# MAGIC-SCAN/adipose_tissue-unet

Measured on AMD Instinct MI355X. Metric: 1024^2 tiles/sec (train), higher is better.
Workload: dtype bf16; 1 GPU; unet_bn L5 base64 1024x1024x3 bf16 B=4/GPU (BASELINE configs[2]); preset=unet_bn, levels=5, tile=1024, batch_per_gpu=4, global_batch=4, parallelism=dp1

## Files before the change

adipose_tissue-unet_amd/csrc/conv_common.h:

```cpp
#pragma once
#include "workspace.h"

struct FwdArgs {
  const void* srcA; const void* srcB;
  const float* scA; const float* shA;
  const float* scB; const float* shB;
  int CAs, CBs;
  int Nimg, Hs, Ws;
  int up;
  int Ho, Wo, stride;
  int kh, kw, dil, pad;
  const void* W; int Kpad; int K;
  const float* bias;
  int Nout;
  int relu;
  uint32_t drop_seed; float drop_rate;
  void* out; int out_stride; int out_mode; int Cps;
  void* out2; int out2_stride; int split_c;
  const void* addend; int addend_stride;
  const void* mask; int mask_stride; float mask_scale;
  const void* mask2; int mask2_stride; float mask2_scale;
  float* accum; int accum_stride;
  float* bn_sum; float* bn_sq;
  const void* bnr_z; int bnr_zs;
// ... 197 lines not shown
    }
    Grp<TO> gr;
    if (a.out_mode == 1) {
      int sub = n / a.Cps, c = n - sub * a.Cps;
      int nimg = m / HWo, rem = m - nimg * HWo, yo = rem / a.Wo, xo = rem - yo * a.Wo;
      size_t pix = ((size_t)nimg * (2 * a.Ho) + 2 * yo + (sub >> 1)) * (2 * a.Wo) + 2 * xo + (sub & 1);
      if constexpr (F8) {
        if (a.out_f8) {
          *reinterpret_cast<uint2*>(reinterpret_cast<unsigned char*>(a.out) + pix * a.out_stride + c) = f8x8_from_f(v);
          continue;
        }
      }
      grp_from_f(gr, v);
      grp_store(gr, reinterpret_cast<TO*>(a.out) + pix * a.out_stride + c);
    } else if (a.out_mode == 2 && n >= a.split_c) {
      const int c = n - a.split_c;
      if (a.mask2) {
        float mk[8];
        grp_load(gr, reinterpret_cast<const TO*>(a.mask2) + (size_t)m * a.mask2_stride + c);
        grp_to_f(gr, mk);
#pragma unroll
        for (int j = 0; j < 8; ++j) v[j] = mk[j] > 0.f ? v[j] * a.mask2_scale : 0.f;
      }
      grp_from_f(gr, v);
      grp_store(gr, reinterpret_cast<TO*>(a.out2) + (size_t)m * a.out2_stride + c);
      if (a.bn_sum) {
#pragma unroll
        for (int j = 0; j < 8; ++j) { bs[j] += v[j]; bq[j] += v[j] * v[j]; }
      }
      continue;
    } else {
      if (!a.out) continue;
      if constexpr (F8) {
        if (a.out_f8) {
          *reinterpret_cast<uint2*>(reinterpret_cast<unsigned char*>(a.out) + (size_t)m * a.out_stride + n) =
              f8x8_from_f(v);
          continue;
        }
      }
      float f[8];
      if (a.addend) {
        grp_load(gr, reinterpret_cast<const TO*>(a.addend) + (size_t)m * a.addend_stride + n);
        grp_to_f(gr, f);
#pragma unroll
        for (int j = 0; j < 8; ++j) v[j] += f[j];
      }
      if (a.mask) {
        grp_load(gr, reinterpret_cast<const TO*>(a.mask) + (size_t)m * a.mask_stride + n);
        grp_to_f(gr, f);
#pragma unroll
        for (int j = 0; j < 8; ++j) v[j] = f[j] > 0.f ? v[j] * a.mask_scale : 0.f;
      }
      grp_from_f(gr, v);
      grp_store(gr, reinterpret_cast<TO*>(a.out) + (size_t)m * a.out_stride + n);
      if (a.accum) {
        float* ap = a.accum + (size_t)m * a.accum_stride + n;
        float r[8];
        grp_to_f(gr, r);
#pragma unroll
        for (int j = 0; j < 8; ++j) ap[j] += r[j];
      }
    }
    if (a.bn_sum) {
#pragma unroll
      for (int j = 0; j < 8; ++j) { bs[j] += v[j]; bq[j] += v[j] * v[j]; }
    }
  }
}

template <int NTH, int BN, typename TO = bf16>
ADP_DEV void epi_rows_bnr(const FwdArgs& a, const float* tile, int rows, int m0, int n0, int tid,
                          float (&bs)[8], float (&bq)[8]) {
  constexpr int LT = BN + 4;
  constexpr int GPR = BN / 8;
  constexpr int RSTEP = NTH / GPR;
  const int cg = tid % GPR;
  const int n = n0 + cg * 8;
  if (n >= a.Nout) return;
  for (int row = tid / GPR; row < rows; row += RSTEP) {
    const int m = m0 + row;
    if (m >= a.M) break;
    float v[8], f[8];
    const float4* tp = reinterpret_cast<const float4*>(tile + row * LT + cg * 8);
    float4 t0 = tp[0], t1 = tp[1];
    v[0] = t0.x; v[1] = t0.y; v[2] = t0.z; v[3] = t0.w; v[4] = t1.x; v[5] = t1.y; v[6] = t1.z; v[7] = t1.w;
    Grp<TO> gr;
    if (a.addend) {
      grp_load(gr, reinterpret_cast<const TO*>(a.addend) + (size_t)m * a.addend_stride + n);
      grp_to_f(gr, f);
#pragma unroll
      for (int j = 0; j < 8; ++j) v[j] += f[j];
    }
    if (a.mask) {
      grp_load(gr, reinterpret_cast<const TO*>(a.mask) + (size_t)m * a.mask_stride + n);
      grp_to_f(gr, f);
#pragma unroll
      for (int j = 0; j < 8; ++j) v[j] = f[j] > 0.f ? v[j] * a.mask_scale : 0.f;
    }
    grp_from_f(gr, v);
    grp_store(gr, reinterpret_cast<TO*>(a.out) + (size_t)m * a.out_stride + n);
    grp_to_f(gr, v);
    if (ADP_DBG(a) & 8192) grp_zero(gr);
    else grp_load(gr, reinterpret_cast<const TO*>(a.bnr_z) + (size_t)m * a.bnr_zs + n);
    grp_to_f(gr, f);
    if (ADP_DBG(a) & 16384) continue;
#pragma unroll
    for (int h = 0; h < 2; ++h) {
      const float4 sc = *reinterpret_cast<const float4*>(a.bnr_sc + n + 4 * h);
      const float4 sh = *reinterpret_cast<const float4*>(a.bnr_sh + n + 4 * h);
      const float4 mu = *reinterpret_cast<const float4*>(a.bnr_mean + n + 4 * h);
      const float4 is = *reinterpret_cast<const float4*>(a.bnr_invstd + n + 4 * h);
      const float scv[4] = {sc.x, sc.y, sc.z, sc.w}, shv[4] = {sh.x, sh.y, sh.z, sh.w};
      const float muv[4] = {mu.x, mu.y, mu.z, mu.w}, isv[4] = {is.x, is.y, is.z, is.w};
#pragma unroll
      for (int j = 0; j < 4; ++j) {
        const int jj = 4 * h + j;
        const float db = fmaf(f[jj], scv[j], shv[j]) > 0.f ? v[jj] : 0.f;
        bs[jj] += db;
        bq[jj] += db * (f[jj] - muv[j]) * isv[j];
      }
    }
  }
}

template <int NTH, int BN>
ADP_DEV void epi_bn_flush(const FwdArgs& a, float* red, int n0, int tid, const float (&bs)[8],
                          const float (&bq)[8]) {
  constexpr int GPR = BN / 8;
  if (ADP_DBG(a) & 2) return;
  ADP_LDS_BARRIER();
#pragma unroll
  for (int j = 0; j < 8; ++j) { red[tid * 16 + j] = bs[j]; red[tid * 16 + 8 + j] = bq[j]; }
  ADP_LDS_BARRIER();
  if (tid < BN) {
    const int gg = tid >> 3, j = tid & 7;
    float s = 0.f, q = 0.f;
    for (int t = gg; t < NTH; t += GPR) { s += red[t * 16 + j]; q += red[t * 16 + 8 + j]; }
    const int nn = n0 + tid;
    if (nn < a.Nout) {
      const int c = a.out_mode == 1 ? nn % a.Cps : nn;
      const unsigned blk = blockIdx.x + blockIdx.y * gridDim.x;
      double* rep = a.stat + (size_t)(blk & (adp::STAT_REPL - 1)) * 2 * adp::STAT_CMAX;
      atomicAdd(rep + c, (double)s);
      atomicAdd(rep + adp::STAT_CMAX + c, (double)q);
    }
  }
}

}

namespace adp {
int launch_fwd_tap64(FwdArgs& a, hipStream_t s);
int launch_fwd_tap64p(FwdArgs& a, hipStream_t s, int tile);
int launch_fwd_halo(FwdArgs& a, hipStream_t s);
int launch_fwd_w4(FwdArgs& a, hipStream_t s);
int launch_fwd_cin8(FwdArgs& a, hipStream_t s);
int launch_fwd_cin8_f32(FwdArgs& a, hipStream_t s);
int launch_fwd_halop_f8(FwdArgs& a, hipStream_t s);
int launch_wgrad_tap64(WgradArgs& a, hipStream_t s);
int launch_wgrad_f32(WgradArgs& a, hipStream_t s);
bool wgrad_bna_fusable(const WgradArgs& a);
}
```

adipose_tissue-unet_amd/csrc/conv_igemm.hip:

```cpp
#include "conv_common.h"
#include <type_traits>

namespace {

constexpr int BM = 128, BN = 64, BK = 32, NT = 256;

template <typename T> struct LdsTr;
template <> struct LdsTr<bf16> { static constexpr int LDK = BK + 8; };
template <> struct LdsTr<float> { static constexpr int LDK = BK + 4; };


template <typename T>
ADP_DEV void load_a_group(const FwdArgs& a, Grp<T>& g, bool rowvalid, int n, int ybase, int xbase,
                          int tap, int ci, int k) {
  grp_zero(g);
  if (!rowvalid || k >= a.K) return;
  int ty = tap / a.kw, tx = tap - ty * a.kw;
  int yi = ybase + ty * a.dil - a.pad;
  int xi = xbase + tx * a.dil - a.pad;
  int Hv = a.Hs * a.up, Wv = a.Ws * a.up;
  if (yi < 0 || xi < 0 || yi >= Hv || xi >= Wv) return;
  if (a.up == 2) { yi >>= 1; xi >>= 1; }
  size_t pix = ((size_t)n * a.Hs + yi) * a.Ws + xi;
  const float* sc; const float* sh;
// ... 898 lines not shown
      Grp<T> gr;
      float f[8];
      grp_load(gr, x + m * stride + g * 8);
      grp_to_f(gr, f);
#pragma unroll
      for (int j = 0; j < 8; ++j) s[j] += f[j];
    }
  }
  __shared__ float red[NT * 8];
#pragma unroll
  for (int j = 0; j < 8; ++j) red[threadIdx.x * 8 + j] = s[j];
  __syncthreads();
  for (int c = threadIdx.x; c < C; c += NT) {
    float t = 0.f;
    for (int l = 0; l < lanes; ++l) t += red[(l * G + (c >> 3)) * 8 + (c & 7)];
    if (part) out[(size_t)blockIdx.x * C + c] = t;
    else atomicAdd(out + (fold ? c % fold : c), t);
  }
}

template <typename T>
void launch_bias_grad(const WgradArgs& a, hipStream_t s) {
  const size_t Mp = a.dy_mode == 0 ? (size_t)a.M : (size_t)a.M * 4;
  const int C = a.dy_mode == 0 ? a.Nout : a.Cps;
  const int G = C / 8, lanes = NT / G;
  const int blocks = (int)std::min<size_t>((Mp + lanes - 1) / lanes, 1024);
  const adp::Slabs part = adp::option("wgrad_det", 1) && C % 4 == 0
                              ? adp::reduce_part(adp::Slot::BiasRows, (size_t)blocks * C * sizeof(float), s)
                              : adp::Slabs{};
  hipLaunchKernelGGL(channel_sum_kernel<T>, dim3(blocks), dim3(NT), 0, s, Mp, C, a.dy_stride,
                     reinterpret_cast<const T*>(a.dY), part.p ? part.p : a.dB, 0, part.p ? 1 : 0);
  if (part.p) adp::slab_reduce(blocks, (size_t)C / 4, part, a.dB, s);
}

}

#include "../../include/adipose_hip.h"

namespace {
template <typename T>
int launch_fwd_plain(FwdArgs& a, hipStream_t s, int fast);

void fill_fwd_args(const adp_conv_desc* d, const adp_conv_io* io, FwdArgs& a) {
  a = FwdArgs{};
  a.srcA = io->srcA; a.srcB = io->srcB;
  a.scA = io->bn_scaleA; a.shA = io->bn_shiftA; a.scB = io->bn_scaleB; a.shB = io->bn_shiftB;
  a.CAs = d->CA_stride; a.CBs = d->CB_stride;
  a.Nimg = d->N; a.Hs = d->Hs; a.Ws = d->Ws; a.up = d->upsample ? 2 : 1;
  a.Ho = d->Ho; a.Wo = d->Wo; a.stride = d->stride;
  a.kh = d->kh; a.kw = d->kw; a.dil = d->dil; a.pad = d->pad;
  a.W = io->W; a.K = d->kh * d->kw * (d->CA_stride + d->CB_stride); a.Kpad = (a.K + 31) / 32 * 32;
  a.bias = io->bias; a.Nout = d->Nout; a.relu = d->relu;
  a.drop_seed = d->dropout_seed; a.drop_rate = d->dropout_rate;
  a.out = io->out; a.out_stride = d->out_stride; a.out_mode = d->out_mode; a.Cps = d->shuffle_c;
  a.out2 = io->out2; a.out2_stride = d->out2_stride; a.split_c = d->split_c;
  a.addend = io->addend; a.addend_stride = d->out_stride;
  a.mask = io->mask; a.mask_stride = d->mask_stride; a.mask_scale = d->mask_scale;
  a.mask2 = io->mask2; a.mask2_stride = d->mask2_stride; a.mask2_scale = d->mask2_scale;
  a.accum = io->accum; a.accum_stride = d->accum_stride;
  a.bn_sum = io->bn_sum; a.bn_sq = io->bn_sqsum;
  a.defer_fold = d->bn_defer_fold && io->bn_sum && !io->bnr_z;
  a.bnr_z = io->bnr_z; a.bnr_zs = d->bnr_stride;
  a.bnr_sc = io->bnr_scale; a.bnr_sh = io->bnr_shift; a.bnr_mean = io->bnr_mean; a.bnr_invstd = io->bnr_invstd;
  a.bnr_dgamma = io->bnr_dgamma; a.bnr_dbeta = io->bnr_dbeta;
  a.M = d->N * d->Ho * d->Wo;
  a.debug_flags = adp::option("fwd_debug", 0);
  a.f32 = 0;
  a.stat = (a.bn_sum || a.bnr_z) ? adp::stat_scratch() : nullptr;
  a.act_out = io->act_outA;
  a.ca_real = d->CA_real;
  auto tail48 = [](int stride, int real) { return stride == 64 && real > 0 && real <= 48; };
  a.ztail = (tail48(d->CA_stride, d->CA_real) && (d->CB_stride == 0 || tail48(d->CB_stride, d->CB_real)) ? 1 : 0) |
            (tail48(d->Nout, d->Nout_real) && d->out_mode == 0 ? 2 : 0);
}

int fold_stats(const FwdArgs& a, hipStream_t s) {
  if (!a.stat) return 0;
  if (a.defer_fold)
    return adp::defer_fold_begin(a.out_mode == 1 ? a.Cps : a.Nout, a.bn_sum, s);
  const int C = a.out_mode == 1 ? a.Cps : a.Nout;
  if (a.bnr_z) return adp::stat_fold(C, a.bnr_dbeta, a.bnr_dgamma, s);
  return adp::stat_fold(C, a.bn_sum, a.bn_sq, s);
}

int launch_fwd_f8(const adp_conv_desc* d, const adp_conv_io* io, hipStream_t s) {
  FwdArgs a;
  fill_fwd_args(d, io, a);
  a.f8 = 1;
  a.wscale = io->w_scale;
  a.out_f8 = d->out_fp8;
  ADP_REQUIRE(a.wscale && a.M > 0 && a.Nout > 0 && a.Nout % 8 == 0, "adp_conv_fwd(fp8): needs w_scale and Nout % 8 == 0");
  ADP_REQUIRE(!a.scA && !a.scB && !a.addend && !a.mask && !a.accum && !a.bn_sum && !a.bnr_z && a.drop_rate == 0.f &&
                  (d->out_mode == 0 || d->out_mode == 1) && a.out,
              "adp_conv_fwd(fp8): plain or pixel-shuffle store only (no BN / addend / mask / accum / dropout)");
  ADP_REQUIRE(d->out_mode != 1 || (d->shuffle_c > 0 && d->Nout % d->shuffle_c == 0), "adp_conv_fwd: bad shuffle_c");
  if (a.CAs == 64 && a.CBs % 64 == 0 && adp::launch_fwd_halop_f8(a, s)) {
    adp::kernel_end();
    return adp::check_launch("adp_conv_fwd");
  }
  ADP_REQUIRE(a.CAs % 128 == 0 && a.CBs % 128 == 0,
              "adp_conv_fwd(fp8): source channel strides must be multiples of 128 (one 128-channel K step per tap)");
  if (!adp::launch_fwd_tap64(a, s)) {
    adp::set_error("adp_conv_fwd(fp8): no fp8 kernel for this geometry (needs K == taps * Cin_s, K % 128 == 0)");
    return -1;
  }
  adp::kernel_end();
  return adp::check_launch("adp_conv_fwd");
}

template <typename T>
int launch_fwd(const adp_conv_desc* d, const adp_conv_io* io, hipStream_t s) {
  FwdArgs a;
  fill_fwd_args(d, io, a);
  ADP_REQUIRE(a.CAs % 8 == 0 && a.CBs % 8 == 0, "adp_conv_fwd: channel strides must be multiples of 8");
  if (d->out_fp8) {
    ADP_REQUIRE((std::is_same<T, bf16>::value), "adp_conv_fwd: out_fp8 needs a bf16 or fp8 launch");
    a.out_f8 = 1;
    if (!adp::launch_fwd_cin8(a, s)) {
      adp::set_error("adp_conv_fwd: out_fp8 on a bf16 launch: input layers only (one 8-channel source, Nout == 64, "
                     "no statistics)");
      return -1;
    }
    adp::kernel_end();
    return adp::check_launch("adp_conv_fwd");
  }
  ADP_REQUIRE(a.M > 0 && a.Nout > 0, "adp_conv_fwd: empty problem");
  ADP_REQUIRE(d->out_mode != 1 || (d->shuffle_c > 0 && d->Nout % d->shuffle_c == 0), "adp_conv_fwd: bad shuffle_c");
  ADP_REQUIRE(d->out_mode != 2 || (io->out2 && d->split_c > 0), "adp_conv_fwd: split store needs out2/split_c");
  ADP_REQUIRE(!a.bnr_z || (d->out_mode == 0 && !a.bn_sum && a.bnr_sc && a.bnr_sh && a.bnr_mean && a.bnr_invstd &&
                           a.bnr_dgamma && a.bnr_dbeta && a.bnr_zs == a.out_stride && a.bnr_zs % 8 == 0 &&
                           a.Nout % 8 == 0),
              "adp_conv_fwd: fused BN-backward reduction needs out_mode 0, all bnr_* pointers, z stride == out stride");
  ADP_REQUIRE(!(a.bn_sum || a.bnr_z) || a.stat,
              std::string("adp_conv_fwd: BatchNorm accumulator replicas unavailable: ") + adp_last_error());
  ADP_REQUIRE(!a.stat || (d->out_mode == 1 ? d->shuffle_c : d->Nout) <= adp::STAT_CMAX,
              "adp_conv_fwd: BatchNorm sums need <= 2048 channels");
  const int fast = adp::option("conv_fast", 2);
  if (a.act_out) {
    ADP_REQUIRE(a.scA && a.shA && !a.scB && a.CBs == 0 && io->srcA != io->act_outA,
                "adp_conv_fwd: act_outA needs bn_scaleA / bn_shiftA, one source and its own buffer");
    if (std::is_same<T, bf16>::value && fast == 2 && adp::launch_fwd_halo(a, s)) {
      adp::kernel_end();
      if (adp::check_launch("adp_conv_fwd")) return -2;
      return fold_stats(a, s);
    }
    const int rc = adp_bn_apply(std::is_same<T, bf16>::value ? ADP_BF16 : ADP_F32, (size_t)a.Nimg * a.Hs * a.Ws, a.CAs,
                                a.srcA, a.scA, a.shA, a.act_out, (adp_stream_t)s);
    if (rc) return rc;
    a.srcA = a.act_out;
    a.scA = a.shA = nullptr;
    a.act_out = nullptr;
  }
  if (std::is_same<T, bf16>::value && fast == 2 && !a.scA && !a.scB &&
      (adp::launch_fwd_cin8(a, s) || adp::launch_fwd_halo(a, s) || adp::launch_fwd_tap64(a, s))) {
    adp::kernel_end();
    if (adp::check_launch("adp_conv_fwd")) return -2;
    return fold_stats(a, s);
  }
  if (std::is_same<T, float>::value && fast == 2 && !a.scA && !a.scB) {
    a.f32 = 1;
    if (adp::launch_fwd_cin8_f32(a, s) || adp::launch_fwd_tap64(a, s)) {
      adp::kernel_end();
      if (adp::check_launch("adp_conv_fwd")) return -2;
      return fold_stats(a, s);
    }
    a.f32 = 0;
  }
  const FwdArgs bnr = a;
  a.bnr_z = nullptr;
  if (!a.bn_sum) a.stat = nullptr;
  const int rc = launch_fwd_plain<T>(a, s, fast);
  if (rc != 0) return rc;
  if (a.stat && fold_stats(a, s) != 0) return -2;
  if (!bnr.bnr_z) return 0;
  return adp_bn_bwd_reduce(std::is_same<T, bf16>::value ? ADP_BF16 : ADP_F32, (size_t)bnr.M, bnr.out_stride, bnr.out,
                           bnr.bnr_z, bnr.bnr_sc, bnr.bnr_sh, bnr.bnr_mean, bnr.bnr_invstd, bnr.bnr_dgamma,
                           bnr.bnr_dbeta, (adp_stream_t)s);
}

template <typename T>
int launch_fwd_plain(FwdArgs& a, hipStream_t s, int fast) {
  if (std::is_same<T, bf16>::value && fast == 2 && !a.scA && !a.scB) {
    const int w64 = (a.Nout + 63) / 64 * 64 - a.Nout, w128 = (a.Nout + 127) / 128 * 128 - a.Nout;
    if (a.Nout > 64 && w128 <= w64) {
      a.ntile_n = (a.Nout + 127) / 128;
      a.nblocks = ((a.M + 127) / 128) * a.ntile_n;
      adp::set_kernel("igemm_fwd_glds_kernel<128, 128>");
      hipLaunchKernelGGL((igemm_fwd_glds_kernel<128, 128>), dim3(a.nblocks), dim3(NT), 0, s, a);
    } else {
      a.ntile_n = (a.Nout + 63) / 64;
      a.nblocks = ((a.M + 255) / 256) * a.ntile_n;
      adp::set_kernel("igemm_fwd_glds_kernel<256, 64>");
      hipLaunchKernelGGL((igemm_fwd_glds_kernel<256, 64>), dim3(a.nblocks), dim3(NT), 0, s, a);
    }
    adp::kernel_end();
    return adp::check_launch("adp_conv_fwd");
  }
  if (std::is_same<T, bf16>::value && fast >= 1) {
    const int w64 = (a.Nout + 63) / 64 * 64 - a.Nout, w128 = (a.Nout + 127) / 128 * 128 - a.Nout;
    if (a.Nout > 64 && w128 <= w64) {
      a.ntile_n = (a.Nout + 127) / 128;
      a.nblocks = ((a.M + 127) / 128) * a.ntile_n;
      adp::set_kernel("igemm_fwd_bf16_kernel<128, 128>");
      hipLaunchKernelGGL((igemm_fwd_bf16_kernel<128, 128>), dim3(a.nblocks), dim3(NT), 0, s, a);
    } else {
      a.ntile_n = (a.Nout + 63) / 64;
      a.nblocks = ((a.M + 255) / 256) * a.ntile_n;
      adp::set_kernel("igemm_fwd_bf16_kernel<256, 64>");
      hipLaunchKernelGGL((igemm_fwd_bf16_kernel<256, 64>), dim3(a.nblocks), dim3(NT), 0, s, a);
    }
    adp::kernel_end();
    return adp::check_launch("adp_conv_fwd");
  }
  a.ntile_n = (a.Nout + BN - 1) / BN;
  const int ntm = (a.M + BM - 1) / BM;
  a.nblocks = ntm * a.ntile_n;
  adp::set_kernel(std::is_same<T, bf16>::value ? "igemm_fwd_kernel<bf16>" : "igemm_fwd_kernel<float>");
  hipLaunchKernelGGL(igemm_fwd_kernel<T>, dim3(a.nblocks), dim3(NT), 0, s, a);
  adp::kernel_end();
  return adp::check_launch("adp_conv_fwd");
}

template <typename T>
int launch_wgrad(const adp_conv_desc* d, const adp_conv_io* io, const void* dY, int dy_stride,
                 float* dW, float* dB, hipStream_t s, const adp_bn_bwd_args* bn = nullptr) {
  WgradArgs a{};
  a.srcA = io->srcA; a.srcB = io->srcB;
  a.scA = io->bn_scaleA; a.shA = io->bn_shiftA; a.scB = io->bn_scaleB; a.shB = io->bn_shiftB;
  a.CAs = d->CA_stride; a.CBs = d->CB_stride; a.Nimg = d->N; a.Hs = d->Hs; a.Ws = d->Ws;
  a.up = d->upsample ? 2 : 1; a.Ho = d->Ho; a.Wo = d->Wo; a.stride = d->stride;
  a.kh = d->kh; a.kw = d->kw; a.dil = d->dil; a.pad = d->pad;
  a.K = d->kh * d->kw * (d->CA_stride + d->CB_stride); a.Kpad = (a.K + 31) / 32 * 32;
  a.dY = dY; a.dy_stride = dy_stride; a.dy_mode = d->out_mode == 1 ? 1 : 0; a.Cps = d->shuffle_c;
  a.Nout = d->Nout; a.dW = dW; a.dB = dB;
  a.M = d->N * d->Ho * d->Wo;
  a.ca_real = d->CA_real; a.cb_real = d->CB_real; a.nout_real = d->Nout_real;
  ADP_REQUIRE(a.CAs % 8 == 0 && a.CBs % 8 == 0 && a.Nout % 8 == 0,
              "adp_conv_wgrad: channel strides and Nout must be multiples of 8");
  ADP_REQUIRE(d->out_mode != 2, "adp_conv_wgrad: split-store descriptors are dgrad-only");
  if (bn) {
    a.bna_dA = bn->dA; a.bna_z = bn->z;
    a.bna_sc = bn->scale; a.bna_sh = bn->shift; a.bna_mean = bn->mean; a.bna_invstd = bn->invstd;
    a.bna_gamma = bn->gamma; a.bna_dgamma = bn->dgamma; a.bna_dbeta = bn->dbeta;
    a.bna_inv_count = 1.f / bn->count;
    if (!(std::is_same<T, bf16>::value && adp::option("conv_fast", 2) == 2 && adp::wgrad_bna_fusable(a))) {
      a.bna_dA = nullptr;
      if (!dY) {
        dY = adp::scratch(adp::Slot::UnfusedDz, (size_t)a.M * dy_stride * (std::is_same<T, bf16>::value ? 2 : 4), s);
        if (!dY) return -2;
        a.dY = dY;
      }
      if (adp_bn_bwd_apply(std::is_same<T, bf16>::value ? ADP_BF16 : ADP_F32, (size_t)a.M, dy_stride, bn->dA, bn->z,
                           bn->scale, bn->shift, bn->mean, bn->invstd, bn->gamma, bn->dgamma, bn->dbeta, bn->count,
                           const_cast<void*>(dY), s))
        return -2;
    }
  }
  if (std::is_same<T, bf16>::value && adp::option("conv_fast", 2) == 2 && !a.scA && !a.scB) {
    if (!adp::launch_wgrad_tap64(a, s)) {
      if (a.bna_dA) {
        a.bna_dA = nullptr;
        if (!dY) {
          dY = adp::scratch(adp::Slot::UnfusedDz, (size_t)a.M * dy_stride * 2, s);
          if (!dY) return -2;
          a.dY = dY;
        }
        if (adp_bn_bwd_apply(ADP_BF16, (size_t)a.M, dy_stride, bn->dA, bn->z, bn->scale, bn->shift, bn->mean,
                             bn->invstd, bn->gamma, bn->dgamma, bn->dbeta, bn->count, const_cast<void*>(dY), s))
          return -2;
      }
      const int TN = (a.Nout <= 64 && adp::option("wgrad_glds_tn64", 1)) ? 64 : 128, TK = TN == 64 ? 256 : 128;
      a.ntile_k = (a.K + TK - 1) / TK;
      a.ntile_n = (a.Nout + TN - 1) / TN;
      const int tiles = a.ntile_k * a.ntile_n;
      int splits = (2048 + tiles - 1) / tiles;
      const int maxsplit = (a.M + 511) / 512;
      splits = std::max(1, std::min(splits, maxsplit));
      a.mchunk = ((a.M + splits - 1) / splits + 63) / 64 * 64;
      splits = (a.M + a.mchunk - 1) / a.mchunk;
      if (TN == 64)
        { adp::set_kernel("igemm_wgrad_glds_kernel<64, 256>");
          hipLaunchKernelGGL((igemm_wgrad_glds_kernel<64, 256>), dim3(tiles, splits), dim3(NT), 0, s, a); }
      else
        { adp::set_kernel("igemm_wgrad_glds_kernel<128, 128>");
          hipLaunchKernelGGL((igemm_wgrad_glds_kernel<128, 128>), dim3(tiles, splits), dim3(NT), 0, s, a); }
    }
    adp::kernel_end();
    if (a.dB) launch_bias_grad<bf16>(a, s);
    return adp::check_launch("adp_conv_wgrad");
  }
  if (std::is_same<T, bf16>::value && adp::option("conv_fast", 2) >= 1) {
    const int TN = (a.Nout <= 64 && adp::option("wgrad_tn64", 0)) ? 64 : 128, TK = TN == 64 ? 256 : 128;
    a.ntile_k = (a.K + TK - 1) / TK;
    a.ntile_n = (a.Nout + TN - 1) / TN;
    const int tiles = a.ntile_k * a.ntile_n;
    int splits = (1536 + tiles - 1) / tiles;
    const int maxsplit = (a.M + 511) / 512;
    splits = std::max(1, std::min(splits, maxsplit));
    a.mchunk = ((a.M + splits - 1) / splits + 63) / 64 * 64;
    splits = (a.M + a.mchunk - 1) / a.mchunk;
    if (TN == 64)
      { adp::set_kernel("igemm_wgrad_bf16_kernel<64, 256>");
        hipLaunchKernelGGL((igemm_wgrad_bf16_kernel<64, 256>), dim3(tiles, splits), dim3(NT), 0, s, a); }
    else
      { adp::set_kernel("igemm_wgrad_bf16_kernel<128, 128>");
        hipLaunchKernelGGL((igemm_wgrad_bf16_kernel<128, 128>), dim3(tiles, splits), dim3(NT), 0, s, a); }
    adp::kernel_end();
// ... 60 lines not shown
```

Before: 180.0 tiles/s.

## Add persistent streaming MFMA kernel for transposed-conv forward and dgrad

Adds a dedicated persistent kernel for 2x2 transposed-convolution style GEMMs: 1x1 conv with pixel-shuffle output (forward) and 2x2 stride-2 gather (its data gradient, optionally fused with BN-ReLU backward statistics). The kernel keeps the weight panel resident in LDS or registers, streams activation tiles through a 5-8 stage buffer_load_lds pipeline with manual vmcnt waits, and writes shuffled output directly with permlane swaps. It is dispatched ahead of the generic tap64 path when shapes qualify, aiming to cut weight reloads and memory latency stalls. It adds considerable hand-tuned asm and shape restrictions.

```diff
diff --git a/adipose_tissue-unet_amd/csrc/conv_common.h b/adipose_tissue-unet_amd/csrc/conv_common.h
--- a/adipose_tissue-unet_amd/csrc/conv_common.h
+++ b/adipose_tissue-unet_amd/csrc/conv_common.h
@@ -373,6 +373,7 @@
 namespace adp {
 int launch_fwd_tap64(FwdArgs& a, hipStream_t s);
 int launch_fwd_tap64p(FwdArgs& a, hipStream_t s, int tile);
+int launch_fwd_convt_stream(FwdArgs& a, hipStream_t s);
 int launch_fwd_halo(FwdArgs& a, hipStream_t s);
 int launch_fwd_w4(FwdArgs& a, hipStream_t s);
 int launch_fwd_cin8(FwdArgs& a, hipStream_t s);
diff --git a/adipose_tissue-unet_amd/csrc/conv_convt_stream.hip b/adipose_tissue-unet_amd/csrc/conv_convt_stream.hip
--- /dev/null
+++ b/adipose_tissue-unet_amd/csrc/conv_convt_stream.hip
@@ -0,0 +1,425 @@
+#include "conv_common.h"
+
+namespace {
+
+constexpr unsigned S_OOB = 0x80000000u;
+constexpr int S_RSRC3 = 0x00020000;
+constexpr int S_PANEL = 65536;
+typedef unsigned int s_v2u32 __attribute__((ext_vector_type(2)));
+typedef unsigned int s_v4u32 __attribute__((ext_vector_type(4)));
+typedef __bf16 s_bf16x4 __attribute__((ext_vector_type(4)));
+
+__device__ __forceinline__ void s_lds16(__amdgpu_buffer_rsrc_t r, void* lds, unsigned off) {
+  __builtin_amdgcn_raw_ptr_buffer_load_lds(r, (lds_void*)lds, 16, off, 0, 0, 0);
+}
+__device__ __forceinline__ float4 s_lds_f4(const float* p) {
+  float4 r;
+  const unsigned addr = (unsigned)(uintptr_t)(const __attribute__((address_space(3))) void*)p;
+  asm volatile("ds_read_b128 %0, %1\n\ts_waitcnt lgkmcnt(0)" : "=v"(r) : "v"(addr) : "memory");
+  return r;
+}
+__device__ __forceinline__ void s_lds_add(double* p, float v) {
+  const unsigned addr = (unsigned)(uintptr_t)(__attribute__((address_space(3))) void*)p;
+  const double d = (double)v;
+  asm volatile("ds_add_f64 %0, %1" ::"v"(addr), "v"(d) : "memory");
+}
+#define S_BAR()                            \
+  do {                                     \
+    asm volatile("" ::: "memory");         \
+    __builtin_amdgcn_s_barrier();          \
+    asm volatile("" ::: "memory");         \
+  } while (0)
+
+#define S_W(n) case n: asm volatile("s_waitcnt vmcnt(" #n ")" ::: "memory"); break;
+__device__ __forceinline__ void s_wait_vm(int n) {
+  switch (n) {
+    S_W(0) S_W(1) S_W(2) S_W(3) S_W(4) S_W(5) S_W(6) S_W(7) S_W(8) S_W(9) S_W(10) S_W(11) S_W(12) S_W(13) S_W(14)
+    S_W(15) S_W(16) S_W(17) S_W(18) S_W(19) S_W(20) S_W(21) S_W(22) S_W(23) S_W(24) S_W(25) S_W(26) S_W(27) S_W(28)
+    S_W(29) S_W(30) S_W(31)
+    default:
+      if (n > 31) asm volatile("s_waitcnt vmcnt(32)" ::: "memory");
+      else asm volatile("s_waitcnt vmcnt(0)" ::: "memory");
+  }
+}
+#undef S_W
+
+template <int BN, int BM, int NST, int WNK>
+constexpr int convt_stream_lds() {
+  return (WNK ? 0 : S_PANEL) + NST * BM * 128 + 5 * BN * 4 + 2 * BN * 8;
+}
+
+template <int BN, int BM, int NST, bool BNR, int SUB = 1, int WNK = 0>
+__global__ __launch_bounds__(512, 1) void convt_stream_kernel(FwdArgs a) {
+  constexpr int NTH = 512, ROWB = 128;
+  constexpr int WN = BN / 64, WM = 8 / WN, TM = BM / WM, MI = TM / 16;
+  static_assert(WN * WM == 8 && TM % 16 == 0 && MI >= 1, "wave layout");
+  constexpr int GA = BM * 8 / NTH;
+  static_assert(GA >= 1 && BM % 64 == 0, "staging split");
+  constexpr int STAGE = BM * ROWB;
+  constexpr int MT = SUB * MI, EPI_OPS = 2 * MI;
+  __shared__ __attribute__((aligned(1024))) unsigned char smem[convt_stream_lds<BN, BM, NST, WNK>()];
+  constexpr int OR = WNK ? 0 : S_PANEL, OC = OR + NST * STAGE;
+  float (*cst)[BN] = reinterpret_cast<float (*)[BN]>(smem + OC);
+  double (*sacc)[BN] = reinterpret_cast<double (*)[BN]>(smem + OC + 5 * BN * 4);
+
+  const int tid = threadIdx.x, lane = tid & 63, wave = tid >> 6;
+  const int wr = wave / WN, wc = wave % WN;
+  const int G = gridDim.x;
+  const int lin = xcd_remap(blockIdx.x, G);
+  const int ntiles = a.nblocks, ntn = a.ntile_n, col = lin % ntn;
+  const int mine = lin < ntiles ? (ntiles - lin + G - 1) / G : 0;
+  if (mine == 0) return;
+  const int n0 = col * BN;
+  const int pos = lane & 7;
+  const int HWo = a.Ho * a.Wo;
+  const int nk = a.K / 64, nch = a.CAs / 64;
+  const bool dgrad = a.kh == 2;
+  if (tid < BN) {
+    const int n = n0 + tid;
+    cst[0][tid] = (!BNR && a.bias) ? a.bias[a.out_mode == 1 ? n % a.Cps : n] : 0.f;
+    cst[1][tid] = BNR ? a.bnr_sc[n] : 0.f;
+    cst[2][tid] = BNR ? a.bnr_sh[n] : 0.f;
+    cst[3][tid] = BNR ? a.bnr_mean[n] : 0.f;
+    cst[4][tid] = BNR ? a.bnr_invstd[n] : 0.f;
+    sacc[0][tid] = 0.0;
+    sacc[1][tid] = 0.0;
+  }
+  const int npix = a.Nimg * a.Hs * a.Ws;
+  const __amdgpu_buffer_rsrc_t rsA = __builtin_amdgcn_make_buffer_rsrc((void*)a.srcA, 0, npix * a.CAs * 2, S_RSRC3);
+  const __amdgpu_buffer_rsrc_t rsW = __builtin_amdgcn_make_buffer_rsrc((void*)a.W, 0, a.Nout * a.Kpad * 2, S_RSRC3);
+
+  int tot = 0;
+  if constexpr (WNK == 0) {
+    const int np = BN * nk / 64;
+    for (int j = 0; j < np; ++j) {
+      const int idx = j * NTH + tid;
+      const int kt = idx / (BN * 8), r = (idx >> 3) % BN;
+      const unsigned off = (unsigned)((n0 + r) * a.Kpad * 2 + kt * ROWB + 16 * (pos ^ swz(r)));
+      s_lds16(rsW, smem + (size_t)(j * NTH + wave * 64) * 16, off);
+    }
+    tot += np;
+  }
+
+  unsigned ro[GA];
+  const int rc = 16 * (pos ^ ((tid >> 4) & 7));
+  auto setup_rows = [&](int m0, int h) {
+#pragma unroll
+    for (int i = 0; i < GA; ++i) {
+      const int q = i * (NTH / 8) + (tid >> 3);
+      const int m = m0 + (q / TM) * (SUB * TM) + h * TM + q % TM;
+      int p = m;
+      if (dgrad) {
+        const int img = m / HWo, rem = m - img * HWo, yo = rem / a.Wo, xo = rem - yo * a.Wo;
+        p = (img * a.Hs + 2 * yo) * a.Ws + 2 * xo;
+      }
+      ro[i] = m < a.M ? (unsigned)(p * a.CAs * 2 + rc) : S_OOB;
+    }
+  };
+  auto tile_id = [&](int k) { return k < mine ? lin / ntn + k * (G / ntn) : -1; };
+  int lk = 0, lt = 0, lkt = 0, ls = 0, lk_tile = -1;
+  int mk[NST];
+#pragma unroll
+  for (int i = 0; i < NST; ++i) mk[i] = 0;
+  auto load_next = [&]() {
+    if (lt == 0) lk_tile = tile_id(lk);
+    if (lk_tile < 0) return;
+    if (lkt == 0) setup_rows(lk_tile * (SUB * BM), lt / nk);
+    unsigned d = (unsigned)lkt * ROWB;
+    if (dgrad) {
+      const int tap = lkt / nch, ch = lkt - tap * nch;
+      d = (unsigned)((((tap >> 1) * a.Ws + (tap & 1)) * a.CAs + ch * 64) * 2);
+    }
+    unsigned char* dst = smem + OR + ls * STAGE + wave * 8 * ROWB;
+#pragma unroll
+    for (int i = 0; i < GA; ++i) s_lds16(rsA, dst + i * (NTH / 8) * ROWB, ro[i] + d);
+    tot += GA;
+#pragma unroll
+    for (int i = 0; i < NST; ++i)
+      if (ls == i) mk[i] = tot;
+    ls = ls == NST - 1 ? 0 : ls + 1;
+    if (++lkt == nk) lkt = 0;
+    if (++lt == SUB * nk) { lt = 0; ++lk; }
+  };
+
+  const int r16 = lane & 15, h4 = lane >> 4;
+  f32x4 acc[MT][4];
+  bf16x8 wreg[WNK ? WNK : 1][4][2];
+  auto read_w = [&](int kt, bf16x8 (&fb)[4][2]) {
+    const unsigned char* pb = smem + kt * (BN * ROWB);
+#pragma unroll
+    for (int nt = 0; nt < 4; ++nt)
+#pragma unroll
+      for (int s = 0; s < 2; ++s) {
+        const int q = wc * 64 + nt * 16 + r16, c = 4 * s + h4;
+        fb[nt][s] = *reinterpret_cast<const bf16x8*>(pb + q * ROWB + ((c ^ swz(q)) << 4));
+      }
+  };
+  if constexpr (WNK > 0) {
+#pragma unroll
+    for (int kt = 0; kt < WNK; ++kt)
+#pragma unroll
+      for (int nt = 0; nt < 4; ++nt)
+#pragma unroll
+        for (int s = 0; s < 2; ++s)
+          wreg[kt][nt][s] = __builtin_bit_cast(bf16x8, __builtin_amdgcn_raw_buffer_load_b128(
+              rsW, (unsigned)((n0 + wc * 64 + nt * 16 + r16) * a.Kpad * 2 + kt * ROWB + 16 * (4 * s + h4)), 0, 0));
+  }
+  auto compute = [&](int buf, int kt, int h) {
+    bf16x8 fbl[4][2];
+    if constexpr (WNK == 0) read_w(kt, fbl);
+    const bf16x8 (&fb)[4][2] = WNK ? wreg[WNK ? kt : 0] : fbl;
+    const unsigned char* pa = smem + OR + buf * STAGE;
+#pragma unroll
+    for (int mi = 0; mi < MI; ++mi) {
+      bf16x8 fa[2];
+#pragma unroll
+      for (int s = 0; s < 2; ++s) {
+        const int q = wr * TM + mi * 16 + r16, c = 4 * s + h4;
+        fa[s] = *reinterpret_cast<const bf16x8*>(pa + q * ROWB + ((c ^ swz(q)) << 4));
+      }
+      prio_hi<ADP_PRIO_FWD>();
+#pragma unroll
+      for (int s = 0; s < 2; ++s)
+#pragma unroll
+        for (int nt = 0; nt < 4; ++nt)
+          acc[h * MI + mi][nt] = __builtin_amdgcn_mfma_f32_16x16x32_bf16(fb[nt][s], fa[s], acc[h * MI + mi][nt], 0, 0, 0);
+      prio_lo<ADP_PRIO_FWD>();
+    }
+  };
+
+  const bool shuffle = a.out_mode == 1;
+  const int Hq = 2 * a.Ho, Wq = 2 * a.Wo;
+  const unsigned out_bytes = (shuffle ? (unsigned)(a.Nimg * Hq * Wq) : (unsigned)a.M) * a.out_stride * 2;
+  const __amdgpu_buffer_rsrc_t rsO = __builtin_amdgcn_make_buffer_rsrc(a.out, 0, (int)out_bytes, S_RSRC3);
+  const __amdgpu_buffer_rsrc_t rsZ =
+      __builtin_amdgcn_make_buffer_rsrc((void*)(BNR ? a.bnr_z : a.out), 0, BNR ? a.M * a.bnr_zs * 2 : 0, S_RSRC3);
+  s_v4u32 zr[BNR ? MI : 1][2];
+  auto load_z = [&](int m0, int h) {
+    int tidv = tid;
+    asm volatile("" : "+v"(tidv));
+    const int r16 = tidv & 15, h4 = (tidv >> 4) & 3, wr = (tidv >> 6) / WN, wc = (tidv >> 6) % WN;
+#pragma unroll
+    for (int mt = 0; mt < MI; ++mt) {
+      const int m = m0 + wr * (SUB * TM) + (h * MI + mt) * 16 + r16;
+#pragma unroll
+      for (int pi = 0; pi < 2; ++pi) {
+        const int cw = n0 + wc * 64 + 16 * (2 * pi + (h4 & 1)) + 8 * (h4 >> 1);
+        zr[mt][pi] = __builtin_amdgcn_raw_buffer_load_b128(rsZ, m < a.M ? (unsigned)((m * a.bnr_zs + cw) * 2) : S_OOB, 0, 0);
+      }
+    }
+  };
+  float s1[2][8] = {}, s2[2][8] = {};
+  auto epilogue = [&](int m0, int h) {
+    int tidv = tid;
+    asm volatile("" : "+v"(tidv));
+    const int r16 = tidv & 15, h4 = (tidv >> 4) & 3, wr = (tidv >> 6) / WN, wc = (tidv >> 6) % WN;
+    float bias[4][4];
+    if constexpr (!BNR) {
+#pragma unroll
+      for (int nt = 0; nt < 4; ++nt) {
+        const float4 b4 = s_lds_f4(&cst[0][wc * 64 + nt * 16 + 4 * h4]);
+        bias[nt][0] = b4.x; bias[nt][1] = b4.y; bias[nt][2] = b4.z; bias[nt][3] = b4.w;
+      }
+    }
+    int cqp[2], subp[2], clp[2];
+#pragma unroll
+    for (int pi = 0; pi < 2; ++pi) {
+      clp[pi] = wc * 64 + 16 * (2 * pi + (h4 & 1)) + 8 * (h4 >> 1);
+      const int cw = n0 + clp[pi];
+      subp[pi] = 0;
+      cqp[pi] = cw;
+      if (shuffle) { subp[pi] = cw / a.Cps; cqp[pi] = cw - subp[pi] * a.Cps; }
+    }
+    float kc[BNR ? 2 : 1][4][8];
+    if constexpr (BNR) {
+#pragma unroll
+      for (int pi = 0; pi < 2; ++pi)
+#pragma unroll
+        for (int f = 0; f < 4; ++f)
+#pragma unroll
+          for (int h = 0; h < 2; ++h) {
+            const float4 v = s_lds_f4(&cst[1 + f][clp[pi] + 4 * h]);
+            kc[pi][f][4 * h] = v.x; kc[pi][f][4 * h + 1] = v.y; kc[pi][f][4 * h + 2] = v.z; kc[pi][f][4 * h + 3] = v.w;
+          }
+    }
+#pragma unroll
+    for (int mi = 0; mi < MI; ++mi) {
+      const int mt = h * MI + mi;
+      const int m = m0 + wr * (SUB * TM) + mt * 16 + r16;
+      const bool mv = m < a.M;
+      int img = 0, yo = 0, xo = 0;
+      if (shuffle) {
+        img = m / HWo;
+        const int rem = m - img * HWo;
+        yo = rem / a.Wo;
+        xo = rem - yo * a.Wo;
+      }
+#pragma unroll
+      for (int pi = 0; pi < 2; ++pi) {
+        s_v2u32 o2[2];
+#pragma unroll
+        for (int j = 0; j < 2; ++j) {
+          const int nt = 2 * pi + j;
+          s_bf16x4 o;
+#pragma unroll
+          for (int r = 0; r < 4; ++r) {
+            float x = acc[mt][nt][r];
+            if constexpr (!BNR) {
+              x += bias[nt][r];
+              if (a.relu) x = fmaxf(x, 0.f);
+            }
+            o[r] = (bf16)x;
+          }
+          o2[j] = __builtin_bit_cast(s_v2u32, o);
+        }
+        const auto e0 = __builtin_amdgcn_permlane16_swap(o2[0].x, o2[1].x, false, false);
+        const auto e1 = __builtin_amdgcn_permlane16_swap(o2[0].y, o2[1].y, false, false);
+        const s_v4u32 st = {e0[0], e1[0], e0[1], e1[1]};
+        int pixo = m;
+        if (shuffle) pixo = (img * Hq + 2 * yo + (subp[pi] >> 1)) * Wq + 2 * xo + (subp[pi] & 1);
+        const unsigned off = mv ? (unsigned)((pixo * a.out_stride + cqp[pi]) * 2) : S_OOB;
+        __builtin_amdgcn_raw_buffer_store_b128(st, rsO, off, 0, 0);
+        if constexpr (BNR) {
+          const bf16x8 g8 = __builtin_bit_cast(bf16x8, st), z8 = __builtin_bit_cast(bf16x8, zr[mi][pi]);
+#pragma unroll
+          for (int e = 0; e < 8; ++e) {
+            const float g = (float)g8[e], zf = (float)z8[e];
+            const float db = fmaf(zf, kc[pi][0][e], kc[pi][1][e]) > 0.f ? g : 0.f;
+            s1[pi][e] += db;
+            s2[pi][e] += db * (zf - kc[pi][2][e]) * kc[pi][3][e];
+          }
+        }
+      }
+    }
+    if (BNR && h == SUB - 1) {
+#pragma unroll
+      for (int pi = 0; pi < 2; ++pi) {
+#pragma unroll
+        for (int e = 0; e < 8; ++e) {
+          s1[pi][e] = row16_sum(s1[pi][e]);
+          s2[pi][e] = row16_sum(s2[pi][e]);
+        }
+        if (r16 == 0) {
+#pragma unroll
+          for (int e = 0; e < 8; ++e) {
+            s_lds_add(&sacc[0][clp[pi] + e], s1[pi][e]);
+            s_lds_add(&sacc[1][clp[pi] + e], s2[pi][e]);
+          }
+        }
+#pragma unroll
+        for (int e = 0; e < 8; ++e) s1[pi][e] = s2[pi][e] = 0.f;
+      }
+    }
+  };
+
+#pragma unroll
+  for (int i = 0; i < NST - 1; ++i) load_next();
+  int cs = 0;
+  for (int k = 0;; ++k) {
+    const int tk = tile_id(k);
+    if (tk < 0) break;
+    const int m0c = tk * (SUB * BM);
+#pragma unroll
+    for (int i = 0; i < MT; ++i)
+#pragma unroll
+      for (int j = 0; j < 4; ++j) acc[i][j] = f32x4{0.f, 0.f, 0.f, 0.f};
+#pragma unroll
+    for (int h = 0; h < SUB; ++h) {
+#define S_KSTEP(t_)                                                                                                   \
+  do {                                                                                                                \
+    int mkc = mk[0];                                                                                                  \
+    _Pragma("unroll") for (int i = 1; i < NST; ++i) if (cs == i) mkc = mk[i];                                        \
+    s_wait_vm(tot - mkc);                                                                                             \
+    S_BAR();  \
+    if constexpr (BNR) {                                                                                              \
+      if ((t_) == 0) {                                                                                                \
+        load_z(m0c, h);                                                                                               \
+        tot += EPI_OPS;                                                                                               \
+      }                                                                                                               \
+    }                                                                                                                 \
+    load_next();                                                                                                      \
+    compute(cs, (t_), h);                                                                                             \
+    cs = cs == NST - 1 ? 0 : cs + 1;                                                                                  \
+  } while (0)
+    if constexpr (WNK > 0) {
+#pragma unroll
+      for (int t = 0; t < WNK; ++t) S_KSTEP(t);
+    } else {
+      for (int t = 0; t < nk; ++t) S_KSTEP(t);
+    }
+#undef S_KSTEP
+    epilogue(m0c, h);
+    tot += EPI_OPS;
+    }
+  }
+
+  if constexpr (BNR) {
+    asm volatile("s_waitcnt lgkmcnt(0)" ::: "memory");
+    __syncthreads();
+    double* rep = a.stat + (size_t)(blockIdx.x & (adp::STAT_REPL - 1)) * 2 * adp::STAT_CMAX;
+    if (tid < BN) {
+      atomicAdd(rep + n0 + tid, sacc[0][tid]);
+      atomicAdd(rep + adp::STAT_CMAX + n0 + tid, sacc[1][tid]);
+    }
+  }
+}
+
+#undef S_BAR
+
+}
+
+namespace adp {
+int launch_fwd_convt_stream(FwdArgs& a, hipStream_t s) {
+  const int mode = option("convt_stream", 2);
+  if (!mode) return 0;
+  constexpr int UNSET = -7654321;
+  if (mode != 1 && (option("fwd_tap64", UNSET) != UNSET || option("tap64_persist", UNSET) != UNSET ||
+                    option("tap64p_cfg", UNSET) != UNSET))
+    return 0;
+  if (a.f32 || a.f8 || a.out_f8) return 0;
+  if (a.addend || a.mask || a.mask2 || a.accum || a.drop_rate > 0.f || a.scA || a.scB || a.bn_sum || a.act_out) return 0;
+  if (a.CBs != 0 || a.up != 1 || a.pad != 0 || !a.out) return 0;
+  if (option("tap64p_claim", option("dp_claim", 0))) return 0;
+  const bool fwd = a.kh == 1 && a.kw == 1 && a.stride == 1 && a.out_mode == 1 && !a.bnr_z && a.Ho == a.Hs &&
+                   a.Wo == a.Ws && a.Cps > 0 && a.Cps % 16 == 0 && a.Nout == 4 * a.Cps;
+  const bool dgr = a.kh == 2 && a.kw == 2 && a.stride == 2 && a.dil == 1 && a.out_mode == 0 && a.Hs == 2 * a.Ho &&
+                   a.Ws == 2 * a.Wo && a.Nout % 64 == 0 && (!a.bnr_z || (!a.bias && !a.relu && a.bnr_zs % 8 == 0));
+  if (!fwd && !dgr) return 0;
+  if (a.CAs % 64 != 0 || a.K != a.kh * a.kw * a.CAs || a.Kpad != a.K || a.K > 512 || a.out_stride % 8 != 0) return 0;
+  const size_t lim = (size_t)1 << 31, pix = (size_t)a.Nimg * a.Hs * a.Ws;
+  const size_t outb = (size_t)a.M * (fwd ? 4 : 1) * a.out_stride * 2;
+  if (pix * a.CAs * 2 >= lim || outb >= lim || (size_t)a.Nout * a.Kpad * 2 >= lim ||
+      (a.bnr_z && (size_t)a.M * a.bnr_zs * 2 >= lim))
+    return 0;
+  int BN = 0;
+  for (int bn : {256, 128, 64})
+    if (!BN && a.Nout % bn == 0 && bn * a.K * 2 <= S_PANEL) BN = bn;
+  if (!BN) return 0;
+  const int wnk = fwd && a.Nout == 512 && a.K == 256 && option("convt_stream_wreg", 1) ? 4 : 0;
+  if (wnk) BN = 512;
+  if (mode != 1 && (a.Nout != BN || a.K > 256 || (dgr && !a.bnr_z))) return 0;
+  constexpr int BM = 128, NST = 5;
+  const bool bnr = a.bnr_z != nullptr;
+  const int sub = bnr && BN == 128 ? 2 : 1;
+  a.ntile_n = a.Nout / BN;
+  const int bm = wnk ? 64 : BM;
+  a.nblocks = (a.M + sub * bm - 1) / (sub * bm) * a.ntile_n;
+  int grid = std::min(a.nblocks, option("tap64_persist_grid", 256));
+  grid -= grid % a.ntile_n;
+  if (grid <= 0) grid = a.ntile_n;
+  set_kernel(bnr ? "convt_stream_kernel<%d, %d, %d, true, %d, %d>" : "convt_stream_kernel<%d, %d, %d, false, %d, %d>", BN,
+             bm, wnk ? 8 : NST, sub, wnk);
+#define S_LAUNCH(BN_)                                                                                          \
+  do {                                                                                                         \
+    if (bnr) hipLaunchKernelGGL((convt_stream_kernel<BN_, BM, NST, true, (BN_ == 128 ? 2 : 1)>), dim3(grid),   \
+                                dim3(512), 0, s, a);                                                          \
+    else hipLaunchKernelGGL((convt_stream_kernel<BN_, BM, NST, false>), dim3(grid), dim3(512), 0, s, a);      \
+  } while (0)
+  if (wnk) hipLaunchKernelGGL((convt_stream_kernel<512, 64, 8, false, 1, 4>), dim3(grid), dim3(512), 0, s, a);
+  else if (BN == 256) S_LAUNCH(256);
+  else if (BN == 128) S_LAUNCH(128);
+  else S_LAUNCH(64);
+#undef S_LAUNCH
+  return 1;
+}
+}
diff --git a/adipose_tissue-unet_amd/csrc/conv_igemm.hip b/adipose_tissue-unet_amd/csrc/conv_igemm.hip
--- a/adipose_tissue-unet_amd/csrc/conv_igemm.hip
+++ b/adipose_tissue-unet_amd/csrc/conv_igemm.hip
@@ -1074,7 +1074,8 @@
     a.act_out = nullptr;
   }
   if (std::is_same<T, bf16>::value && fast == 2 && !a.scA && !a.scB &&
-      (adp::launch_fwd_cin8(a, s) || adp::launch_fwd_halo(a, s) || adp::launch_fwd_tap64(a, s))) {
+      (adp::launch_fwd_cin8(a, s) || adp::launch_fwd_halo(a, s) || adp::launch_fwd_convt_stream(a, s) ||
+       adp::launch_fwd_tap64(a, s))) {
     adp::kernel_end();
     if (adp::check_launch("adp_conv_fwd")) return -2;
     return fold_stats(a, s);
```

Result: no change. 178.5 tiles/s (-0.8%).
